# furcelay/gigalens

Hardware: AMD Instinct MI355X
Metric: forward+grad lens sims/sec, 128x128 px batch 1024; achieved HBM GB/s vs peak (higher is better)
Workload: dtype f32; 1 GPU; C2: EPL+shear lens, Sersic source, 128x128 px, batch 1024 per GPU, fp32 (BASELINE.json configs[1]); samples_per_gpu=1024, pixels=16384, z_dim=13, mode=fwdgrad, parallelism=single GPU

## Files before the change

### gigalens_amd/csrc/gigalens_hip.hip

```cpp
#include "../../include/gigalens_hip.h"

#include <hip/hip_runtime.h>

#include <algorithm>
#include <cmath>
#include <cstdarg>
#include <cstdio>
#include <cstdlib>
#include <cstring>
#include <new>
#include <vector>

#define GL_AUX_KERNELS 1
#include "gl_host_tables.h"
#include "gl_model.h"
#include "gl_static.hip.h"
#include "gl_post.hip.h"
#include "gl_positions.hip.h"
#include "gl_images.hip.h"
#include "gl_potential.hip.h"
#include "gl_lstsq.hip.h"
#include "gl_shp.hip.h"

using namespace glk;

namespace {
thread_local char g_err[512] = "";
}

namespace glk {
int fail(int code, const char* fmt, ...) {
  va_list ap;
  va_start(ap, fmt);
  vsnprintf(g_err, sizeof(g_err), fmt, ap);
  va_end(ap);
  return code;
}
}

namespace {

size_t align_up(size_t v, size_t a) { return (v + a - 1) / a * a; }

int env_int(const char* name, int dflt) {
  const char* s = getenv(name);
  return (s && *s) ? atoi(s) : dflt;
}

}


namespace {

void chunking(const gl_model* m, int B, int* chunk, int* n_chunks) {
  const long long tile_px = (long long)WG * 4;
  long long want = std::max<long long>((768 + B - 1) / B, ((long long)m->N + 8191) / 8192);
  if (m->target_wgs_set || !m->static_id) want = std::max<long long>(1, (m->target_wgs + B - 1) / B);
  long long per = ((long long)m->N + want - 1) / want;
  per = std::max(tile_px, (per + tile_px - 1) / tile_px * tile_px);
  if (m->chunk_px_override > 0) per = m->chunk_px_override;
  *chunk = (int)per;
  *n_chunks = (int)(((long long)m->N + per - 1) / per);
}

bool wave_front_end(const gl_model* m) { return m->has_epl && (int)m->comps.size() <= 64 && m->wave_prep; }
bool order_in_front_end(const gl_model* m, int B) {
  return wave_front_end(m) && m->use_order && m->order_fused && m->epl_comp >= 0 && B >= 2;
}

int tail_plan(const gl_model* m, int B, int n_chunks, int* tail_from, int* n_rows) {
  *tail_from = B;
  *n_rows = n_chunks;
  const bool pair_epl = m->pair && (m->static_id == ST_EPLSHEAR_SERSIC || m->static_id == ST_EPLSHEAR_SERSIC_SERSIC);
  if (m->tail_rows == 0 || !pair_epl || m->has_post || !order_in_front_end(m, B) || B > 1024) return 0;
  const int tiles = (m->N + 2 * WG - 1) / (2 * WG);
  const int slots = 256 * (m->static_id == ST_EPLSHEAR_SERSIC ? 3 : 2);
  int n_tail = m->tail_n, rows = m->tail_rows;
  if (n_tail < 0) {
    const long long wgs = (long long)B * n_chunks, rem = wgs % slots;
    if (wgs < slots || rem * 4 < slots) return 0;
    n_tail = (int)(rem / n_chunks);
  }
  if (rows < 0) rows = 2 * n_chunks;
  if (n_tail <= 0 || n_tail > B || rows > tiles || rows == n_chunks) return 0;
  *tail_from = B - n_tail;
  *n_rows = std::max(n_chunks, rows);
  return rows;
}

struct Workspace {
  float* derived;
  float* partial;
  float* params;
  int* order;
  int* cost;
  float* gal_dyn;
  float *pos_w, *pos_adj, *pos_g, *pos_fam, *pos_ll, *pos_chi2, *pos_grad;
  float* img_ss;
  float* img_tmp;
  float* stats;
  size_t bytes;
};

Workspace carve(const gl_model* m, int B, void* base) {
  int chunk, n_chunks;
  chunking(m, B, &chunk, &n_chunks);
  Workspace w{};
  size_t off = 0;
  char* p = (char*)base;
  w.derived = (float*)(p + off);
  off += align_up((size_t)B * m->D * sizeof(float), 256);
  w.partial = (float*)(p + off);
  int tail_from, n_rows;
  tail_plan(m, B, n_chunks, &tail_from, &n_rows);
  off += align_up((size_t)B * n_rows * m->A * sizeof(float), 256);
  w.params = (float*)(p + off);
  off += align_up((size_t)B * std::max(m->P, 1) * sizeof(float), 256);
  w.order = (int*)(p + off);
  off += align_up((size_t)B * sizeof(int), 256);
  w.cost = (int*)(p + off);
  off += align_up((size_t)B * sizeof(int), 256);
  if (m->G) {
    w.gal_dyn = (float*)(p + off);
    off += align_up((size_t)B * m->G * GM_ND * sizeof(float), 256);
  }
  if (m->pos_J) {
    auto take = [&](size_t n) { float* q = (float*)(p + off); off += align_up(n * sizeof(float), 256); return q; };
    w.pos_w = take((size_t)B * m->pos_J * 6);
    w.pos_adj = take((size_t)B * m->pos_J * 3);
    w.pos_g = take((size_t)B * m->pos_J * std::max(m->P, 1));
    w.pos_fam = take((size_t)B * m->pos_F * 2);
    w.pos_ll = take(B);
    w.pos_chi2 = take(B);
    w.pos_grad = take((size_t)B * std::max(m->P, 1));
  }
  if (m->has_post) {
    w.img_ss = (float*)(p + off);
    off += align_up((size_t)B * m->height * m->width * sizeof(float), 256);
    w.img_tmp = (float*)(p + off);
    off += align_up((size_t)B * (m->height / m->supersample) * (m->width / m->supersample) * sizeof(float), 256);
    w.stats = (float*)(p + off);
    off += align_up((size_t)B * 2 * sizeof(float), 256);
  }
  w.bytes = off;
  return w;
}


MainArgs base_args(const gl_model* m, const Workspace& w, int chunk) {
  MainArgs a{};
  a.comps = m->d_comps;
  a.n_lens = m->n_lens;
  a.n_ll = m->n_ll;
  a.n_src = m->n_src;
  a.derived = w.derived;
  a.D = m->D;
  a.A = m->A;
  a.Apad = m->Apad;
  a.ncols = m->ncols;
// ... 494 lines not shown
    int off = NSTAT;
    bool ok_row = true;
    for (int i = 0; i < n_comp; ++i) {
      ok_row = ok_row && m->comps[i].a_off == off;
      off += static_nacc(m->comps[i].kind);
    }
    if (!ok_row || off != m->A) m->pair = 0;
  }
  {
    int off = NSTAT;
    bool ok_row = true;
    for (int i = 0; i < n_comp; ++i) {
      ok_row = ok_row && m->comps[i].a_off == off;
      off += static_nacc(m->comps[i].kind);
    }
    m->shp_kernel = env_int("GIGALENS_HIP_SHP", 1) && env_int("GIGALENS_HIP_PAIR", 1) && m->static_id && ok_row && n_src == 1 &&
                    m->comps.back().kind == K_SHAPELETS;
  }
  m->light_spherical = n_comp > n_lens;
  for (int i = n_lens; i < n_comp; ++i) m->light_spherical = m->light_spherical && m->comps[i].kind == K_SERSIC;
  if (!m->tile_grad) m->tile_grad = m->static_id ? 1 : 2;
  if (!m->static_id) {
    const bool env_tile = env_int("GIGALENS_HIP_TILE", 0) != 0;
    if (!env_tile && !m->has_epl && !m->has_shapelets && !m->fam) m->tile = 4;
    if (m->tile == 1) m->tile = 2;
    if (m->tile_grad == 1) m->tile_grad = 2;
  }
  if (env_int("GIGALENS_HIP_CLUSTER", 1) && !m->static_id && !m->has_user && n_lens_light == 0 && n_lens >= 1 && n_lens <= 8 && n_src >= 1 &&
      n_src <= 20 && (size_t)64 * m->Apad * sizeof(float) <= 64 * 1024) {
    bool ok_c = true, ell = false;
    for (int i = 0; i < n_lens; ++i) ok_c = ok_c && m->comps[i].kind == K_NFW;
    for (int i = n_lens; i < n_comp; ++i) {
      ok_c = ok_c && (m->comps[i].kind == K_SERSIC || m->comps[i].kind == K_SERSIC_ELLIPSE);
      ell = ell || m->comps[i].kind == K_SERSIC_ELLIPSE;
    }
    constexpr int NFWP = (NFW_ND + 3) & ~3, SERP = (SER_NDX + 3) & ~3;
    for (int i = 0; i < n_lens && ok_c; ++i) ok_c = m->comps[i].d_off == NFWP * i && m->comps[i].a_off == NSTAT + NFW_NACC * i;
    for (int i = 0; i < n_src && ok_c; ++i)
      ok_c = m->comps[n_lens + i].d_off == NFWP * n_lens + SERP * i && m->comps[n_lens + i].a_off == NSTAT + NFW_NACC * n_lens + SER_NACC * i;
    ok_c = ok_c && (size_t)64 * m->Apad * sizeof(float) + sizeof(float) * 2 * glh::kNfwNodes <= 64 * 1024;
    if (ok_c) m->cluster = ell ? 2 : 1;
    if (m->cluster) {
      const int cap = (n_lens <= 4 && n_src <= 8) ? 12 : (n_src <= 12 ? 20 : 28);
      const int mode = env_int("GIGALENS_HIP_CLUSTER", -1);
      m->cluster_w = mode == 2 || (mode != 1 && 10 * (n_lens + n_src) >= 6 * cap);
    }
  }
  m->target_wgs = std::max(1, env_int("GIGALENS_HIP_TARGET_WGS", 2048));
  m->target_wgs_set = getenv("GIGALENS_HIP_TARGET_WGS") != nullptr;
  m->use_order = env_int("GIGALENS_HIP_ORDER", 1) != 0;
  m->order_fused = env_int("GIGALENS_HIP_ORDER_FUSED", 1) != 0;
  m->prep_lds = env_int("GIGALENS_HIP_PREP_LDS", 1) != 0;
  m->tail_rows = env_int("GIGALENS_HIP_TAIL_ROWS", -1);
  m->tail_n = env_int("GIGALENS_HIP_TAIL_N", -1);
#ifdef GL_EXPERIMENTS
  m->chunk_px_override = env_int("GIGALENS_HIP_CHUNK_PX", 0);
  m->dbg_flags = env_int("GIGALENS_HIP_DBGFLAGS", 0);
  if (m->chunk_px_override < 0 || m->chunk_px_override % (WG * 4) != 0) {
    const int bad = m->chunk_px_override;
    delete m;
    return fail(GL_EINVAL, "GIGALENS_HIP_CHUNK_PX=%d is not a positive multiple of the tile (%d pixels)", bad, WG * 4);
  }
  if (m->dbg_flags || m->chunk_px_override)
    fprintf(stderr, "libgigalens_hip: EXPERIMENT BUILD with GIGALENS_HIP_DBGFLAGS=%d GIGALENS_HIP_CHUNK_PX=%d -- results are not valid\n",
            m->dbg_flags, m->chunk_px_override);
#else
  for (const char* name : {"GIGALENS_HIP_DBGFLAGS", "GIGALENS_HIP_CHUNK_PX"}) {
    const char* v = getenv(name);
    if (v && *v && atoi(v) != 0) {
      delete m;
      return fail(GL_EINVAL, "%s is set but this library was built without -DGL_EXPERIMENTS (the dissection knobs do not exist in it)", name);
    }
  }
#endif
  m->shp_cull = env_int("GIGALENS_HIP_SHP_CULL", 1);
  m->shp_blocked = env_int("GIGALENS_HIP_SHP_BLOCKED", 1);
  m->corr_max_pairs = env_int("GIGALENS_HIP_CORR_MAXPAIRS", 0);
  m->corr_wide = env_int("GIGALENS_HIP_CORR_WIDE", 1);
  m->wave_prep = env_int("GIGALENS_HIP_WAVE_PREP", 1) != 0;
  m->lstsq_wgs = std::max(1, env_int("GIGALENS_HIP_LSTSQ_WGS", 2048));
  m->lstsq_chol = env_int("GIGALENS_HIP_LSTSQ_CHOL", 1) != 0;
  m->lstsq_fused = env_int("GIGALENS_HIP_LSTSQ_FUSED", 1) != 0;
  size_t shmem = (size_t)(((m->D + 3) & ~3) + m->ncols * m->Apad) * sizeof(float) + m->nfw_lds;
  if (shmem > 64 * 1024) { delete m; return fail(GL_EUNSUPPORTED, "model needs %zu B of LDS per workgroup (> 64 KiB)", shmem); }

  auto up = [&](void** dst, const void* src, size_t bytes) -> bool {
    if (hipMalloc(dst, bytes) != hipSuccess) return false;
    return hipMemcpy(*dst, src, bytes, hipMemcpyHostToDevice) == hipSuccess;
  };
  bool ok = true;
  if (n_comp) ok = ok && up((void**)&m->d_comps, m->comps.data(), sizeof(CompDesc) * n_comp);
  else ok = ok && (hipMalloc((void**)&m->d_comps, sizeof(CompDesc)) == hipSuccess);
  ok = ok && up((void**)&m->d_gx, grid->grid_x, sizeof(float) * m->N);
  for (int i = 0; i < m->N; ++i) m->grid_rmax = std::max(m->grid_rmax, std::hypot(grid->grid_x[i], grid->grid_y[i]));
  ok = ok && up((void**)&m->d_gy, grid->grid_y, sizeof(float) * m->N);
  if (!m->lin_cols.empty()) ok = ok && up((void**)&m->d_lin_cols, m->lin_cols.data(), sizeof(int) * m->lin_cols.size());
  if (grid->pix_index) {
    for (int i = 0; i < m->N && ok; ++i)
      if (grid->pix_index[i] < 0 || grid->pix_index[i] >= m->height * m->width) {
        gl_model_destroy(m);
        return fail(GL_EINVAL, "pix_index[%d]=%d out of range", i, grid->pix_index[i]);
      }
    ok = ok && up((void**)&m->d_pix, grid->pix_index, sizeof(int) * m->N);
  }
  if (m->has_nfw) {
    std::vector<float> tab;
    glh::build_nfw_table([](double X, double& g, double& gp) { glp::nfw_gw<double>(X, g, gp); }, tab);
    const float neutral_nfw[4] = {0.f, 0.f, 1.f, 0.f};
    float neutral_ser[16] = {0.f};
    neutral_ser[glp::SER_C] = neutral_ser[glp::SER_SQ] = neutral_ser[glp::SER_ISQ] = neutral_ser[glp::SER_INVRS] = 1.f;
    neutral_ser[glp::SER_INVN] = neutral_ser[glp::SER_IRS2] = 1.f;
    neutral_ser[glp::SER_BN] = 1.6721f;
    tab.insert(tab.end(), neutral_nfw, neutral_nfw + 4);
    tab.insert(tab.end(), neutral_ser, neutral_ser + 16);
    std::vector<float> tab_s;
    glh::build_nfw_table_s([](double X, double& g, double& gp) { glp::nfw_gw<double>(X, g, gp); }, tab_s);
    tab.insert(tab.end(), tab_s.begin(), tab_s.end());
    ok = ok && up((void**)&m->d_nfw_tab, tab.data(), tab.size() * sizeof(float));
  }
  if (m->has_table) {
    std::vector<float> tab;
    (void)sh_nmax;
    glh::build_shapelet_table(m->shp_big ? SH_CAPB : SH_CAP, tab, &m->shp_stride);
    ok = ok && up((void**)&m->d_shp_tab, tab.data(), tab.size() * sizeof(float));
  }
  m->has_post = grid->psf != nullptr || grid->supersample != 1;
  if (m->has_post) {
    const int kh = grid->psf ? grid->psf_h : 1, kw = grid->psf ? grid->psf_w : 1, ss = grid->supersample;
    m->psf_h = kh;
    m->psf_w = kw;
    m->KH = kh + ss - 1;
    m->KW = kw + ss - 1;
    m->pad_t = (kh - 1) / 2;
    m->pad_l = (kw - 1) / 2;
    std::vector<double> keff((size_t)m->KH * m->KW, 0.0);
    for (int u = 0; u < kh; ++u)
      for (int v = 0; v < kw; ++v) {
        double f = grid->psf ? (double)grid->psf[(size_t)(kh - 1 - u) * kw + (kw - 1 - v)] : 1.0;
        for (int a2 = 0; a2 < ss; ++a2)
          for (int c2 = 0; c2 < ss; ++c2) keff[(size_t)(u + a2) * m->KW + (v + c2)] += f / (double)(ss * ss);
      }
    std::vector<float> kf(keff.begin(), keff.end());
    ok = ok && up((void**)&m->d_psf, kf.data(), sizeof(float) * kf.size());
    if (env_int("GIGALENS_HIP_CORR_PAIR", 1) && ss <= 2 && m->KW <= 32 && m->KH <= 64) {
      const int Hs = m->height, Ws = m->width, H = Hs / ss, W = Ws / ss;
      std::vector<float> kbuf;
      auto pad4 = [](int n) { return std::max(4, (n + 3) & ~3); };
      {
        gl_model::CorrPlan& f = m->corr_fwd;
        f.KWP = pad4(m->KW);
        f.ST = ss;
        CorrClass c{};
        c.koff = 0; c.KH = m->KH; c.pt = m->pad_t; c.pl = m->pad_l; c.Ho = H; c.Wo[0] = W; c.oo_r = 0; c.oo_c[0] = 0;
        kbuf.assign((size_t)m->KH * f.KWP, 0.f);
        for (int u = 0; u < m->KH; ++u)
          for (int v = 0; v < m->KW; ++v) kbuf[(size_t)u * f.KWP + v] = (float)keff[(size_t)u * m->KW + v];
        f.args.n_class = 1; f.args.ncj = 1; f.args.Hi = Hs; f.args.Wi = Ws; f.args.Hout = H; f.args.Wout = W; f.args.os = 1;
        f.args.cls[0] = c;
        f.max_Ho = H; f.max_Wo = W; f.max_KH = m->KH; f.ok = true;
      }
      {
        gl_model::CorrPlan& g = m->corr_bwd;
        g.ST = 1;
        g.args.n_class = ss; g.args.ncj = ss; g.args.Hi = H; g.args.Wi = W; g.args.Hout = Hs; g.args.Wout = Ws; g.args.os = ss;
        int Cn[4], rjn[4], pln[4], max_pl = -(1 << 30), width = 1;
        for (int pj = 0; pj < ss; ++pj) {
// ... 1118 lines not shown
```

### gigalens_amd/csrc/gl_launch.hip.h

```cpp
#pragma once
#include <hip/hip_ext.h>

#include "gl_model.h"
#include "gl_static.hip.h"
#include "gl_pair.hip.h"
#include "gl_shp.hip.h"

namespace glk {

template <int MODE>
bool launch_static(const gl_model* m, const MainArgs& a, dim3 grid, dim3 block, size_t shmem, hipStream_t stream, hipEvent_t ev0, hipEvent_t ev1) {
  const int T = (MODE == IMG_BWD || MODE == LL_GRAD) ? m->tile_grad : m->tile;
#define GL_PAIR(WW, LK, CK, SK)                                                           \
  do {                                                                                    \
    m->last_main_fn = (const void*)&gl_pair_kernel<MODE, v2f, WW, LK, CK, SK>;            \
    hipExtLaunchKernelGGL((gl_pair_kernel<MODE, v2f, WW, LK, CK, SK>), grid, block, (std::uint32_t)(shmem), stream, ev0, ev1, 0, a); \
  } while (0)
  if (m->pair) {
    constexpr bool G = (MODE == IMG_BWD || MODE == LL_GRAD);
    constexpr int W1 = G ? 3 : 4, W2 = G ? 2 : 4;
    if (m->light_spherical) {
      switch (m->static_id) {
        case ST_EPLSHEAR_SERSIC: GL_PAIR(W1, L_EplShear, C_None, C_Sersic); return true;
        case ST_EPLSHEAR_SERSIC_SERSIC: GL_PAIR(W2, L_EplShear, C_Sersic, C_Sersic); return true;
        case ST_SIE_SERSIC: GL_PAIR(W1, L_Sie, C_None, C_Sersic); return true;
        case ST_SIESHEAR_SERSIC_SERSIC: GL_PAIR(W1, L_SieShear, C_Sersic, C_Sersic); return true;
        default: break;
      }
    } else {
      switch (m->static_id) {
        case ST_EPLSHEAR_SERSIC: GL_PAIR(W1, L_EplShear, C_None, C_SersicE); return true;
        case ST_EPLSHEAR_SERSIC_SERSIC: GL_PAIR(W2, L_EplShear, C_SersicE, C_SersicE); return true;
        case ST_SIE_SERSIC: GL_PAIR(W1, L_Sie, C_None, C_SersicE); return true;
        case ST_SIESHEAR_SERSIC_SERSIC: GL_PAIR(W2, L_SieShear, C_SersicE, C_SersicE); return true;
        default: break;
      }
    }
  }
#undef GL_PAIR
  if (m->shp_kernel && (m->static_id == ST_EPLSHEAR_SHAPELETS || m->static_id == ST_EPLSHEAR_SERSIC_SHAPELETS)) {
    constexpr int NPS = SH_SQ / 2;
    const size_t epi = (size_t)(16 * m->Apad + 4 * 16 * 17) * sizeof(float);
    const size_t sh = (size_t)((m->D + 3) & ~3) * sizeof(float) + std::max(shp_exchange_bytes(NPS), epi);
    const bool interp = (m->comps.back().flags & GL_FLAG_SHAPELETS_INTERPOLATE) != 0;
    const bool ragged = a.mask || a.pix || (a.N % (2 * WG)) != 0 || (a.chunk % (2 * WG)) != 0;
    MainArgs ab = a;
    ab.blk_w = (interp && !ragged && m->shp_blocked && m->width % 16 == 0 && m->height % 8 == 0 &&
                (long long)a.N == (long long)m->width * m->height) ? m->width : 0;
#define GL_SHP2(LLK_, I_, R_)                                                                                 \
  do {                                                                                                        \
    m->last_main_fn = (const void*)&gl_shp_kernel<MODE, 2, L_EplShear, LLK_, NPS, I_, R_>;                     \
    hipExtLaunchKernelGGL((gl_shp_kernel<MODE, 2, L_EplShear, LLK_, NPS, I_, R_>), grid, block, (std::uint32_t)(sh), stream, ev0, ev1, 0, ab);   \
  } while (0)
#define GL_SHP(LLK_, I_) do { if (ragged) GL_SHP2(LLK_, I_, true); else GL_SHP2(LLK_, I_, false); } while (0)
    if (m->static_id == ST_EPLSHEAR_SHAPELETS) { if (interp) GL_SHP(C_None, true); else GL_SHP(C_None, false); }
    else { if (interp) GL_SHP(C_SersicE, true); else GL_SHP(C_SersicE, false); }
#undef GL_SHP
#undef GL_SHP2
    return true;
  }
#define GL_LAUNCH(TT, WW, LK, CK, SK)                                                        \
  do {                                                                                       \
    m->last_main_fn = (const void*)&gl_static_kernel<MODE, TT, WW, LK, CK, SK>;              \
    hipExtLaunchKernelGGL((gl_static_kernel<MODE, TT, WW, LK, CK, SK>), grid, block, (std::uint32_t)(shmem), stream, ev0, ev1, 0, a); \
  } while (0)
  switch (m->static_id) {
    case ST_EPLSHEAR_SERSIC:
      if (T == 4) { if (m->static_variant == 2) GL_LAUNCH(4, 2, L_EplShear, C_None, C_Sersic); else GL_LAUNCH(4, 3, L_EplShear, C_None, C_Sersic); }
      else if (T == 1) GL_LAUNCH(1, 4, L_EplShear, C_None, C_Sersic);
      else { if (m->static_variant == 3) GL_LAUNCH(2, 3, L_EplShear, C_None, C_Sersic); else GL_LAUNCH(2, 4, L_EplShear, C_None, C_Sersic); }
      return true;
    case ST_EPLSHEAR_SERSIC_SERSIC:
      if (T == 4) GL_LAUNCH(4, 2, L_EplShear, C_Sersic, C_Sersic); else GL_LAUNCH(2, 4, L_EplShear, C_Sersic, C_Sersic);
      return true;
    case ST_SIE_SERSIC:
      if (T == 4) GL_LAUNCH(4, 4, L_Sie, C_None, C_Sersic); else GL_LAUNCH(2, 4, L_Sie, C_None, C_Sersic);
      return true;
    case ST_SIESHEAR_SERSIC_SERSIC:
      if (T == 4) GL_LAUNCH(4, 4, L_SieShear, C_Sersic, C_Sersic); else GL_LAUNCH(2, 4, L_SieShear, C_Sersic, C_Sersic);
      return true;
    case ST_EPLSHEAR_SHAPELETS:
      if (T == 2) GL_LAUNCH(2, 2, L_EplShear, C_None, C_Shapelets); else if (T == 1) GL_LAUNCH(1, 2, L_EplShear, C_None, C_Shapelets);
      else return false;
      return true;
    case ST_EPLSHEAR_SERSIC_SHAPELETS:
      if (T == 2) GL_LAUNCH(2, 2, L_EplShear, C_Sersic, C_Shapelets); else if (T == 1) GL_LAUNCH(1, 2, L_EplShear, C_Sersic, C_Shapelets);
      else return false;
      return true;
  }
#undef GL_LAUNCH
  return false;
}

template <int MODE>
int launch_generic(const gl_model* m, const MainArgs& a, dim3 grid, dim3 block, size_t shmem, hipStream_t stream, hipEvent_t ev0, hipEvent_t ev1);

template <int MODE>
int launch_main(const gl_model* m, const MainArgs& a, int B, int n_chunks, hipStream_t stream) {
  dim3 grid(n_chunks, B), block(WG);
  if (a.tail_rows > 0)
    grid.y = a.tail_from + (unsigned)(((long long)(B - a.tail_from) * a.tail_rows + n_chunks - 1) / n_chunks);
  size_t shmem = (size_t)(((m->D + 3) & ~3) + m->ncols * m->Apad) * sizeof(float) + m->nfw_lds;
  const bool timed = m->timing_slots && (m->timing_calls.fetch_add(1) % m->timing_stride) == 0;
// ... 22 lines not shown
```

### gigalens_amd/csrc/gl_pair.hip.h

```cpp
#pragma once
#include "gl_static.hip.h"
#include "gl_vec.hip.h"

namespace glk {

#ifdef GL_HAVE_USER
template <class V, int CODE> __device__ __forceinline__ void user_mass_fwd_v(const float* d, V x, V y, V& bx, V& by) {
  constexpr unsigned body = (unsigned)user_code_body(CODE);
  if constexpr (sizeof(V) == sizeof(float)) {
    float ax, ay;
    glu::mass_fwd(body, d, x, y, ax, ay);
    bx -= ax; by -= ay;
  } else {
    float ax0, ay0, ax1, ay1;
    glu::mass_fwd(body, d, x.x, y.x, ax0, ay0);
    glu::mass_fwd(body, d, x.y, y.y, ax1, ay1);
    bx -= V{ax0, ax1};
    by -= V{ay0, ay1};
  }
}
template <class V, int CODE> __device__ __forceinline__ void user_mass_vjp_v(const float* d, V x, V y, V gx, V gy, V* acc) {
  constexpr unsigned body = (unsigned)user_code_body(CODE);
  constexpr int NPAR = user_code_npar(CODE);
  float t0[NPAR > 0 ? NPAR : 1], t1[NPAR > 0 ? NPAR : 1];
#pragma unroll
  for (int k = 0; k < NPAR; ++k) { t0[k] = 0.f; t1[k] = 0.f; }
  if constexpr (sizeof(V) == sizeof(float)) {
    glu::mass_vjp(body, d, x, y, gx, gy, t0);
#pragma unroll
    for (int k = 0; k < NPAR; ++k) acc[k] += t0[k];
  } else {
    glu::mass_vjp(body, d, x.x, y.x, gx.x, gy.x, t0);
    glu::mass_vjp(body, d, x.y, y.y, gx.y, gy.y, t1);
#pragma unroll
    for (int k = 0; k < NPAR; ++k) acc[k] += V{t0[k], t1[k]};
  }
}
template <class V, int CODE> __device__ __forceinline__ V user_light_fwd_v(const float* d, V x, V y) {
  constexpr unsigned body = (unsigned)user_code_body(CODE);
  if constexpr (sizeof(V) == sizeof(float)) return glu::light_fwd(body, d, x, y);
  else return V{glu::light_fwd(body, d, x.x, y.x), glu::light_fwd(body, d, x.y, y.y)};
}
template <class V, int CODE, bool SRC>
__device__ __forceinline__ void user_light_vjp_v(const float* d, V x, V y, V g, V* acc, V& gpx, V& gpy) {
  constexpr unsigned body = (unsigned)user_code_body(CODE);
  constexpr int NPAR = user_code_npar(CODE);
  float t0[NPAR > 0 ? NPAR : 1], t1[NPAR > 0 ? NPAR : 1];
#pragma unroll
  for (int k = 0; k < NPAR; ++k) { t0[k] = 0.f; t1[k] = 0.f; }
  if constexpr (sizeof(V) == sizeof(float)) {
    float dgx = 0.f, dgy = 0.f;
    glu::light_vjp(body, d, x, y, g, t0, dgx, dgy);
#pragma unroll
    for (int k = 0; k < NPAR; ++k) acc[k] += t0[k];
    if (SRC) { gpx += dgx; gpy += dgy; }
  } else {
    float dgx0 = 0.f, dgy0 = 0.f, dgx1 = 0.f, dgy1 = 0.f;
    glu::light_vjp(body, d, x.x, y.x, g.x, t0, dgx0, dgy0);
    glu::light_vjp(body, d, x.y, y.y, g.y, t1, dgx1, dgy1);
#pragma unroll
    for (int k = 0; k < NPAR; ++k) acc[k] += V{t0[k], t1[k]};
    if (SRC) { gpx += V{dgx0, dgx1}; gpy += V{dgy0, dgy1}; }
  }
}
#endif

template <int MODE, class V, int WAVES, class LK, class LLK, class SK>
__global__ void __launch_bounds__(WG, WAVES) gl_pair_kernel(MainArgs a) {
  constexpr int NL = LK::n, NLL = LLK::n, NS = SK::n, NLIGHT = NLL + NS;
  constexpr bool GRAD = (MODE == IMG_BWD || MODE == LL_GRAD);
  constexpr int W = sizeof(V) / sizeof(float);
  extern __shared__ float smem[];
  float* s_d = smem;
  float* s_acc = smem + ((a.D + 3) & ~3);
  const int tid = threadIdx.x;
  int rank = blockIdx.y, row = blockIdx.x, n_rows = gridDim.x, my_rows = gridDim.x;
  int p0 = row * a.chunk, p1 = min(p0 + a.chunk, a.N);
  if (a.tail_rows > 0) {
    n_rows = a.n_rows;
    if (rank >= a.tail_from) {
      const int j = (rank - a.tail_from) * (int)gridDim.x + row;
      rank = a.tail_from + j / a.tail_rows;
      if (rank >= a.n_samples) return;
      row = j % a.tail_rows;
      my_rows = a.tail_rows;
      const int tiles = (a.N + W * WG - 1) / (W * WG);
      p0 = (int)((long long)row * tiles / a.tail_rows) * (W * WG);
      p1 = min((int)((long long)(row + 1) * tiles / a.tail_rows) * (W * WG), a.N);
    }
  }
  const int b = a.order ? a.order[rank] : rank;
  const CompDesc* __restrict__ comps = a.comps;
  const float* __restrict__ gder = a.derived + (size_t)b * a.D;
  if (!GL_DBG(a.dbg, 4)) {
    if (a.D <= WG) {
      if (tid < a.D) s_d[tid] = gder[tid];
    } else {
      for (int i = tid; i < a.D; i += WG) s_d[i] = gder[i];
    }
  }
  __syncthreads();
  constexpr int NACC_L = [] { int n = 0; for (int i = 0; i < NL; ++i) n += static_nacc(LK::kinds[i]); return n; }();
  constexpr int NACC_C = [] {
    int n = 0;
    for (int i = 0; i < NLL; ++i) n += static_nacc(LLK::kinds[i]);
    for (int i = 0; i < NS; ++i) n += static_nacc(SK::kinds[i]);
    return n;
  }();
  V accL[NACC_L > 0 ? NACC_L : 1];
  V accC[NACC_C > 0 ? NACC_C : 1];
#pragma unroll
  for (int k = 0; k < NACC_L; ++k) accL[k] = V(0.f);
#pragma unroll
  for (int k = 0; k < NACC_C; ++k) accC[k] = V(0.f);
  V st0 = V(0.f), st1 = V(0.f);
  V wsum = V(0.f);
  int n_whole = 0;
  const float* dL[NL > 0 ? NL : 1];
  const float* dC[NLIGHT > 0 ? NLIGHT : 1];
#pragma unroll
  for (int i = 0; i < NL; ++i) dL[i] = s_d + comps[i].d_off;
#pragma unroll
  for (int i = 0; i < NLIGHT; ++i) dC[i] = s_d + comps[NL + i].d_off;
  const bool has_err = a.err != nullptr, has_mask = a.mask != nullptr, has_pix = a.pix != nullptr;

  auto tile = [&](int base, auto check_tag, auto err_tag) {
    constexpr bool CHECK = decltype(check_tag)::value;
    constexpr int ERR = decltype(err_tag)::value;
    const bool herr = ERR == 2 ? has_err : ERR == 1;
    unsigned jj[W], pidx[W];
    bool valid[W];
    V x, y, vmask = V(1.f);
#pragma unroll
    for (int w = 0; w < W; ++w) {
      int j = base + w * WG + tid;
      valid[w] = CHECK ? (j < p1) : true;
      jj[w] = (unsigned)(valid[w] ? j : p1 - 1);
      pidx[w] = (CHECK && has_pix) ? (unsigned)a.pix[jj[w]] : jj[w];
    }
    unsigned jo[W], po[W];
#pragma unroll
    for (int w = 0; w < W; ++w) { jo[w] = jj[w] << 2; po[w] = pidx[w] << 2; }
    auto ldf = [](const float* base, unsigned byte_off) { return *reinterpret_cast<const float*>(reinterpret_cast<const char*>(base) + byte_off); };
    if constexpr (W == 2) {
      x = V{ldf(a.gx, jo[0]), ldf(a.gx, jo[1])};
      y = V{ldf(a.gy, jo[0]), ldf(a.gy, jo[1])};
      if (CHECK) vmask = V{valid[0] ? 1.f : 0.f, valid[1] ? 1.f : 0.f};
    } else {
      x = ldf(a.gx, jo[0]);
      y = ldf(a.gy, jo[0]);
      if (CHECK) vmask = valid[0] ? 1.f : 0.f;
    }
    V bx = x, by = y, m = V(0.f);
    EplStateV<V> est[NL > 0 ? NL : 1];
    SerStateV<V> sst[NLIGHT > 0 ? NLIGHT : 1];
    static_for([&](auto I) {
      constexpr int i = decltype(I)::value;
      constexpr int kind = LK::kinds[i];
      if constexpr (kind == K_EPL) epl_fwd_v<V, GRAD>(dL[i], gder + comps[i].d_off, x, y, bx, by, est[i]);
      else if constexpr (kind == K_SIE) sie_fwd_v<V>(dL[i], x, y, bx, by);
      else if constexpr (kind == K_SHEAR) shear_fwd_v<V>(dL[i], x, y, bx, by);
#ifdef GL_HAVE_USER
      else if constexpr (is_user_code(kind)) user_mass_fwd_v<V, kind>(dL[i], x, y, bx, by);
#endif
      else sis_fwd_v<V>(dL[i], x, y, bx, by);
    }, std::make_integer_sequence<int, NL>{});
    static_for([&](auto I) {
      constexpr int i = decltype(I)::value;
      constexpr bool src = i >= NLL;
      constexpr int lkind = src ? SK::kinds[src ? i - NLL : 0] : LLK::kinds[src ? 0 : i];
      constexpr bool ell = lkind != K_SERSIC;
#ifdef GL_HAVE_USER
      if constexpr (is_user_code(lkind)) m += user_light_fwd_v<V, lkind>(dC[i], src ? bx : x, src ? by : y);
      else
#endif
      m += sersic_fwd_v<V, ell>(dC[i], src ? bx : x, src ? by : y, sst[i]);
    }, std::make_integer_sequence<int, NLIGHT>{});
    auto nanp = m != m;
    m = (nanp ? V(0.f) : m) * a.out_scale;
    if (MODE == IMG_FWD) {
      float* row = a.img + (size_t)b * a.img_stride;
      if constexpr (W == 2) {
        if (valid[0]) row[pidx[0]] = m.x;
        if (valid[1]) row[pidx[1]] = m.y;
      } else {
        if (valid[0]) row[pidx[0]] = m;
      }
      return;
    }
    V gm;
    if (MODE == IMG_BWD) {
      const float* row = a.gimg + (size_t)b * a.img_stride;
      V g;
      if constexpr (W == 2) g = V{row[pidx[0]], row[pidx[1]]}; else g = row[pidx[0]];
      gm = nanp ? V(0.f) : (CHECK ? g * vmask : g) * a.out_scale;
    } else {
      V o, w = vmask, e = V(1.f);
      if constexpr (W == 2) {
        o = V{ldf(a.obs, po[0]), ldf(a.obs, po[1])};
        if (CHECK && has_mask) w = w * V{ldf(a.mask, po[0]), ldf(a.mask, po[1])};
        if (herr) e = V{ldf(a.err, po[0]), ldf(a.err, po[1])};
      } else {
        o = ldf(a.obs, po[0]);
        if (CHECK && has_mask) w = w * ldf(a.mask, po[0]);
        if (herr) e = ldf(a.err, po[0]);
      }
      V dmo = m - o;
      V s2 = herr ? e * e : m * a.inv_t + a.bg2;
      V is2 = rcp(s2);
      V nm = log2_(s2);
      V c2 = __builtin_elementwise_fma(nm, V(0.f), dmo * dmo * is2);
      if (CHECK) {
        auto use = w != V(0.f);
        st0 += use ? c2 * w : V(0.f);
        st1 += use ? nm * w : V(0.f);
        wsum += w;
      } else {
        st0 += c2;
        st1 += nm;
      }
      if (MODE == LL_GRAD) {
        V g = herr ? -(dmo * is2) : (dmo * dmo * is2 - 1.f) * (is2 * (0.5f * a.inv_t)) - dmo * is2;
        gm = nanp ? V(0.f) : (CHECK ? g * w : g) * a.out_scale;
      }
    }
    if constexpr (GRAD) {
      V gbx = V(0.f), gby = V(0.f);
      static_for([&](auto I) {
        constexpr int i = decltype(I)::value;
        constexpr bool src = i >= NLL;
        constexpr int off = [] {
          int n = 0;
          for (int j = 0; j < i; ++j) n += static_nacc(j < NLL ? LLK::kinds[j < NLL ? j : 0] : SK::kinds[j >= NLL ? j - NLL : 0]);
          return n;
        }();
        constexpr int lkind = src ? SK::kinds[src ? i - NLL : 0] : LLK::kinds[src ? 0 : i];
        constexpr bool ell = lkind != K_SERSIC;
#ifdef GL_HAVE_USER
        if constexpr (is_user_code(lkind)) user_light_vjp_v<V, lkind, src>(dC[i], src ? bx : x, src ? by : y, gm, accC + off, gbx, gby);
        else
#endif
        sersic_vjp_v<V, src, ell>(dC[i], sst[i], gm, accC + off, gbx, gby);
      }, std::make_integer_sequence<int, NLIGHT>{});
      gbx = -gbx;
      gby = -gby;
      static_for([&](auto I) {
        constexpr int i = decltype(I)::value;
        constexpr int kind = LK::kinds[i];
        constexpr int off = [] { int n = 0; for (int j = 0; j < i; ++j) n += static_nacc(LK::kinds[j]); return n; }();
        if constexpr (kind == K_EPL) epl_vjp_v<V>(dL[i], gbx, gby, est[i], accL + off);
        else if constexpr (kind == K_SIE) sie_vjp_v<V>(dL[i], x, y, gbx, gby, accL + off);
        else if constexpr (kind == K_SHEAR) shear_vjp_v<V>(x, y, gbx, gby, accL + off);
#ifdef GL_HAVE_USER
        else if constexpr (is_user_code(kind)) user_mass_vjp_v<V, kind>(dL[i], x, y, gbx, gby, accL + off);
#endif
        else sis_vjp_v<V>(dL[i], x, y, gbx, gby, accL + off);
      }, std::make_integer_sequence<int, NL>{});
    }
  };
  {
    const bool plain = !has_mask && !has_pix;
    int base = p0;
    if (GL_DBG(a.dbg, 1)) base = p1;
    if (plain) {
      if (has_err)
        for (; base + WG * W <= p1; base += WG * W, ++n_whole) tile(base, std::false_type{}, std::integral_constant<int, 1>{});
      else
        for (; base + WG * W <= p1; base += WG * W, ++n_whole) tile(base, std::false_type{}, std::integral_constant<int, 0>{});
    }
    for (; base < p1; base += WG * W) tile(base, std::true_type{}, std::integral_constant<int, 2>{});
  }
  if (MODE == IMG_FWD) return;
  auto norm_term = [](float l2sum, float w) { return (l2sum + w * 2.6514961294723187f) * (float)kLn2; };
  float* out = a.partial + ((size_t)b * n_rows + row) * a.A;
  if (row == 0)
    for (int i = my_rows * a.A + tid; i < n_rows * a.A; i += WG) out[i] = 0.f;
  if (!GRAD) {
    for (int i = tid; i < 4 * a.Apad; i += WG) s_acc[i] = 0.f;
    __syncthreads();
  }
  if constexpr (GRAD) {
    constexpr int NV = NSTAT + NACC_L + NACC_C, NVP = (NV + 3) & ~3;
    float vals[NVP];
#pragma unroll
    for (int k = 0; k < NVP; ++k) vals[k] = 0.f;
    vals[0] = (MODE == LL_GRAD) ? hsum(st0) : 0.f;
    vals[1] = (MODE == LL_GRAD) ? norm_term(hsum(st1), hsum(wsum) + (float)(W * n_whole)) : 0.f;
    static_for([&](auto I) {
      constexpr int i = decltype(I)::value;
      constexpr int kind = LK::kinds[i];
      constexpr int off = [] { int n = 0; for (int j = 0; j < i; ++j) n += static_nacc(LK::kinds[j]); return n; }();
      constexpr int G = static_nacc(kind);
      float tmp[G];
#pragma unroll
      for (int k = 0; k < G; ++k) tmp[k] = hsum(accL[off + k]);
      if constexpr (kind == K_EPL) {
        tmp[EPLA_B] = tmp[EPLA_P0] * (dL[i][EPL_TM1] * dL[i][EPL_INVB]);
        tmp[EPLA_P0] *= rcp(dL[i][EPL_P0]);
        const float gxr = tmp[EPLA_CX], gyr = tmp[EPLA_CY], cc = dL[i][EPL_C], ss = dL[i][EPL_S];
        tmp[EPLA_CX] = -(gxr * cc - gyr * ss);
        tmp[EPLA_CY] = -(gxr * ss + gyr * cc);
      }
#pragma unroll
      for (int k = 0; k < G; ++k) vals[NSTAT + off + k] = tmp[k];
    }, std::make_integer_sequence<int, NL>{});
    static_for([&](auto I) {
      constexpr int i = decltype(I)::value;
      constexpr int off = [] {
        int n = 0;
        for (int j = 0; j < i; ++j) n += static_nacc(j < NLL ? LLK::kinds[j < NLL ? j : 0] : SK::kinds[j >= NLL ? j - NLL : 0]);
        return n;
      }();
      constexpr int lkind = i < NLL ? LLK::kinds[i < NLL ? i : 0] : SK::kinds[i >= NLL ? i - NLL : 0];
      if constexpr (is_user_code(lkind)) {
#pragma unroll
        for (int k = 0; k < static_nacc(lkind); ++k) vals[NSTAT + NACC_L + off + k] = hsum(accC[off + k]);
      } else {
#pragma unroll
        for (int k = 0; k < SER_NACC; ++k) vals[NSTAT + NACC_L + off + k] = hsum(accC[off + k]) * (k == SERA_INVN ? (float)kLn2 : 1.f);
      }
    }, std::make_integer_sequence<int, NLIGHT>{});
    const bool odd = tid & 1, hi = tid & 2;
    float* s_row16 = s_acc + (tid >> 4) * a.Apad;
#pragma unroll
    for (int g = 0; g < NVP / 4; ++g) {
      float r = quad_transpose_sum(vals[4 * g], vals[4 * g + 1], vals[4 * g + 2], vals[4 * g + 3], odd, hi);
      r = dpp_add(r, 0x114, 0xF);
      r = dpp_add(r, 0x118, 0xF);
      if ((tid & 15) >= 12 && 4 * g + (tid & 3) < NV) s_row16[4 * g + (tid & 3)] = r;
    }
    __syncthreads();
    for (int k = tid; k < NV; k += WG) {
      float v = 0.f;
#pragma unroll
// ... 22 lines not shown
```

### gigalens_amd/csrc/gl_static.hip.h

```cpp
#pragma once
#if defined(__HIPCC_RTC__) && !__has_include(<utility>)
namespace std {
template <class T, T v> struct integral_constant {
  static constexpr T value = v;
  typedef T value_type;
  typedef integral_constant type;
  constexpr operator T() const { return v; }
};
typedef integral_constant<bool, true> true_type;
typedef integral_constant<bool, false> false_type;
template <class T, T... Is> struct integer_sequence {};
template <class T, T N> using make_integer_sequence = __make_integer_seq<integer_sequence, T, N>;
template <bool B, class T, class F> struct conditional { typedef T type; };
template <class T, class F> struct conditional<false, T, F> { typedef F type; };
template <bool B, class T, class F> using conditional_t = typename conditional<B, T, F>::type;
}
#else
#include <utility>
#endif

#include "gl_kernels.hip.h"
#include "gl_shapelets.hip.h"

namespace glk {
// ... 312 lines not shown
          return n;
        }();
        const float* d = dC[i];
#pragma unroll
        for (int t = 0; t < T; ++t) {
          float dgx = 0.f, dgy = 0.f;
          if constexpr (kind == K_SHAPELETS)
            shp_vjp_state<SH_CAP>(d, gder + comps[NL + i].d_off + SHP_AMP, comps[NL + i].flags & 1u, hst[i][t], gm[t],
                                  accC + off, dgx, dgy);
          else
            sersic_vjp_state(d, sst[i][t], gm[t], accC + off, dgx, dgy);
          if (src) { gbx[t] += dgx; gby[t] += dgy; }
        }
      }, std::make_integer_sequence<int, NLIGHT>{});
#pragma unroll
      for (int t = 0; t < T; ++t) { gbx[t] = -gbx[t]; gby[t] = -gby[t]; }
      static_for([&](auto I) {
        constexpr int i = decltype(I)::value;
        constexpr int kind = LK::kinds[i];
        constexpr int off = [] { int n = 0; for (int j = 0; j < i; ++j) n += static_nacc(LK::kinds[j]); return n; }();
        const float* d = dL[i];
        if constexpr (kind == K_EPL) {
          epl_vjp_state<T>(d, gbx, gby, est[i], accL + off);
        } else {
#pragma unroll
          for (int t = 0; t < T; ++t) {
            if constexpr (kind == K_SIE) sie_vjp(d, x[t], y[t], gbx[t], gby[t], accL + off);
            else if constexpr (kind == K_NFW) nfw_vjp(d, x[t], y[t], gbx[t], gby[t], accL + off);
            else if constexpr (kind == K_SHEAR) shear_vjp(d, x[t], y[t], gbx[t], gby[t], accL + off);
            else sis_vjp(d, x[t], y[t], gbx[t], gby[t], accL + off);
          }
        }
      }, std::make_integer_sequence<int, NL>{});
    }
  }
  if (MODE == IMG_FWD) return;
  const AccCol ac = acc_col(s_acc, a.Apad, a.ncols, tid);
  if (MODE == LL_FWD || MODE == LL_GRAD) wave_acc<2>(st, ac, 0);
  if constexpr (GRAD) {
    static_for([&](auto I) {
      constexpr int i = decltype(I)::value;
      constexpr int off = [] { int n = 0; for (int j = 0; j < i; ++j) n += static_nacc(LK::kinds[j]); return n; }();
      constexpr int G = static_nacc(LK::kinds[i]);
      float tmp[G];
#pragma unroll
      for (int k = 0; k < G; ++k) tmp[k] = accL[off + k];
      wave_acc<G>(tmp, ac, comps[i].a_off, comps[i].n_acc);
    }, std::make_integer_sequence<int, NL>{});
    static_for([&](auto I) {
      constexpr int i = decltype(I)::value;
      constexpr int kind = i < NLL ? LLK::kinds[i < NLL ? i : 0] : SK::kinds[i >= NLL ? i - NLL : 0];
      constexpr int off = [] {
        int n = 0;
        for (int j = 0; j < i; ++j) n += static_nacc(j < NLL ? LLK::kinds[j < NLL ? j : 0] : SK::kinds[j >= NLL ? j - NLL : 0]);
        return n;
      }();
      constexpr int G = static_nacc(kind);
      float tmp[G];
#pragma unroll
      for (int k = 0; k < G; ++k) tmp[k] = accC[off + k];
      wave_acc<G>(tmp, ac, comps[NL + i].a_off, comps[NL + i].n_acc);
    }, std::make_integer_sequence<int, NLIGHT>{});
  }
  __syncthreads();
  float* out = a.partial + ((size_t)b * gridDim.x + chunk) * a.A;
  for (int k = tid; k < a.A; k += WG) {
    float v = 0.f;
    for (int j = 0; j < a.ncols; ++j) v += s_acc[j * a.Apad + k];
    out[k] = v;
  }
}

using L_EplShear = KindList<K_EPL, K_SHEAR>;
using L_Sie = KindList<K_SIE>;
using L_SieShear = KindList<K_SIE, K_SHEAR>;
using C_None = KindList<>;
using C_Sersic = KindList<K_SERSIC>;
using C_SersicE = KindList<K_SERSIC_ELLIPSE>;
using C_Shapelets = KindList<K_SHAPELETS>;

enum StaticId { ST_NONE = 0, ST_EPLSHEAR_SERSIC, ST_EPLSHEAR_SERSIC_SERSIC, ST_SIE_SERSIC, ST_EPLSHEAR_SHAPELETS,
                ST_SIESHEAR_SERSIC_SERSIC, ST_EPLSHEAR_SERSIC_SHAPELETS  };


}
```

### gigalens_amd/csrc/gl_vec.hip.h

```cpp
#pragma once
#include <hip/hip_runtime.h>

#include "gl_profiles.h"

namespace glk {
using namespace glp;

typedef float v2f __attribute__((ext_vector_type(2)));

using glm::rcp;
using glm::sqrt_;
using glm::exp2_;
using glm::log2_;
using glm::atan_;
using glm::atanh_;

__device__ __forceinline__ v2f rcp(v2f a) { return v2f{glm::rcp(a.x), glm::rcp(a.y)}; }
__device__ __forceinline__ v2f sqrt_(v2f a) { return v2f{glm::sqrt_(a.x), glm::sqrt_(a.y)}; }
__device__ __forceinline__ float rsq_(float a) { return __builtin_amdgcn_rsqf(a); }
__device__ __forceinline__ v2f rsq_(v2f a) { return v2f{__builtin_amdgcn_rsqf(a.x), __builtin_amdgcn_rsqf(a.y)}; }
__device__ __forceinline__ v2f exp2_(v2f a) { return v2f{glm::exp2_(a.x), glm::exp2_(a.y)}; }
__device__ __forceinline__ v2f log2_(v2f a) { return v2f{glm::log2_(a.x), glm::log2_(a.y)}; }
__device__ __forceinline__ v2f atan_(v2f a) { return v2f{glm::atan_(a.x), glm::atan_(a.y)}; }
__device__ __forceinline__ v2f atanh_(v2f a) { return v2f{glm::atanh_(a.x), glm::atanh_(a.y)}; }
template <class V> __device__ __forceinline__ V vexp(V x) {
  const float hi = (float)kLog2e;
  const float lo = (float)(kLog2e - (double)(float)kLog2e);
  V t = x * hi;
  V e = __builtin_elementwise_fma(x, V(hi), -t) + x * lo;
  V p = exp2_(t);
  return __builtin_elementwise_fma(p, e * (float)kLn2, p);
}
template <> __device__ __forceinline__ float vexp<float>(float x) { return glm::exp_(x); }
template <class V> __device__ __forceinline__ V vlog(V x) { return log2_(x) * (float)kLn2; }
__device__ __forceinline__ float floor_at(float a, float lo) { return __builtin_fmaxf(a, lo); }
__device__ __forceinline__ v2f floor_at(v2f a, float lo) { return v2f{__builtin_fmaxf(a.x, lo), __builtin_fmaxf(a.y, lo)}; }
__device__ __forceinline__ float clamp3(float a, float lo, float hi) { return __builtin_amdgcn_fmed3f(a, lo, hi); }
__device__ __forceinline__ v2f clamp3(v2f a, float lo, float hi) { return v2f{__builtin_amdgcn_fmed3f(a.x, lo, hi), __builtin_amdgcn_fmed3f(a.y, lo, hi)}; }
template <class V> __device__ __forceinline__ V vmin(V a, V b) { return a < b ? a : b; }
template <class V> __device__ __forceinline__ V vmax(V a, V b) { return a > b ? a : b; }
__device__ __forceinline__ float hsum(float a) { return a; }
__device__ __forceinline__ float hsum(v2f a) { return a.x + a.y; }

template <class V> struct EplStateV {
  V xr, yr, inv, invc, L2, P, Cs, Ss, arx, ary;
  V f0, f1, t0, t1;
};

typedef const float __attribute__((address_space(4)))* gptr4;
typedef float vf4 __attribute__((ext_vector_type(4)));
template <class T, class P> struct gl_rebind;
template <class T> struct gl_rebind<T, const float*> { using type = const T*; };
template <class T> struct gl_rebind<T, gptr4> { using type = const T __attribute__((address_space(4)))*; };

template <class V, bool GRAD, class P = const float*>
__device__ __forceinline__ void epl_fwd_v(const float* d, const P gd, V x, V y, V& bx, V& by,
                                          EplStateV<V>& st) {
  using PInt = typename gl_rebind<int, P>::type;
  using PRow = typename gl_rebind<vf4, P>::type;
  const float c = d[EPL_C], s = d[EPL_S], q = d[EPL_Q];
  V dx = x - d[EPL_CX], dy = y - d[EPL_CY];
  st.xr = dx * c + dy * s;
  st.yr = dy * c - dx * s;
  V X = st.xr * q;
  V r2 = X * X + st.yr * st.yr;
  V r = rsq_(r2);
  auto pos = r2 > V(0.f);
  st.inv = pos ? r : V(0.f);
  st.Cs = pos ? X * r : V(1.f);
  st.Ss = st.yr * st.inv;
  V iRc = clamp3(r, 1e-10f, 1e10f);
  st.invc = (iRc == r) ? r : V(0.f);
  V twoc = (st.Cs * st.Cs - st.Ss * st.Ss) * 2.f;
  const int K = ((PInt)gd)[EPL_KI];
  const PRow gtab = (PRow)(gd + EPL_TAB);
  V o1, o2, f1 = V(0.f), f2 = V(0.f), t1 = V(0.f), t2 = V(0.f);
  auto term = [&](const vf4 ck, V& b1, V& b2, V& g1, V& g2, V& h1, V& h2) {
    b2 = __builtin_elementwise_fma(twoc, b1, V(ck.x)) - b2;
    if (GRAD) {
      g2 = __builtin_elementwise_fma(twoc, g1, V(ck.z)) - g2;
      h2 = __builtin_elementwise_fma(twoc, h1, V(ck.w)) - h2;
    }
  };
  auto four = [&](const vf4 r0, const vf4 r1, const vf4 r2, const vf4 r3) {
    term(r3, o1, o2, f1, f2, t1, t2);
    term(r2, o2, o1, f2, f1, t2, t1);
    term(r1, o1, o2, f1, f2, t1, t2);
    term(r0, o2, o1, f2, f1, t2, t1);
  };
  auto four_first = [&](const vf4 r0, const vf4 r1, const vf4 r2, const vf4 r3) {
    o1 = __builtin_elementwise_fma(twoc, V(r3.x), V(r2.x));
    o2 = __builtin_elementwise_fma(twoc, o1, V(r1.x)) - V(r3.x);
    o1 = __builtin_elementwise_fma(twoc, o2, V(r0.x)) - o1;
    if (GRAD) {
      f1 = __builtin_elementwise_fma(twoc, V(r3.z), V(r2.z));
      f2 = __builtin_elementwise_fma(twoc, f1, V(r1.z)) - V(r3.z);
      f1 = __builtin_elementwise_fma(twoc, f2, V(r0.z)) - f1;
      t1 = __builtin_elementwise_fma(twoc, V(r3.w), V(r2.w));
      t2 = __builtin_elementwise_fma(twoc, t1, V(r1.w)) - V(r3.w);
      t1 = __builtin_elementwise_fma(twoc, t2, V(r0.w)) - t1;
    }
  };
  int trips = (K + 4) >> 2;
  int row = 4 * trips - 4;
  PRow p = gtab + row;
  vf4 a0 = p[0], a1 = p[1], a2 = p[2], a3 = p[3];
  row = row >= 4 ? row - 4 : 0;
  p = gtab + row;
  vf4 b0 = p[0], b1 = p[1], b2 = p[2], b3 = p[3];
  four_first(a0, a1, a2, a3);
  if (--trips != 0) {
    while (true) {
      row = row >= 4 ? row - 4 : 0;
      p = gtab + row;
      a0 = p[0]; a1 = p[1]; a2 = p[2]; a3 = p[3];
      four(b0, b1, b2, b3);
      if (--trips == 0) break;
      row = row >= 4 ? row - 4 : 0;
      p = gtab + row;
      b0 = p[0]; b1 = p[1]; b2 = p[2]; b3 = p[3];
      four(a0, a1, a2, a3);
      if (--trips == 0) break;
    }
  }
  const V o0 = o1, ob = o2;
  if (GRAD) { st.f0 = f1; st.f1 = f2; st.t0 = t1; st.t1 = t2; }
  const V Ox = (o0 - ob) * st.Cs, Oy = (o0 + ob) * st.Ss;
  st.L2 = log2_(iRc * d[EPL_B]);
  st.P = exp2_(st.L2 * d[EPL_TM1]) * d[EPL_P0];
  const V arx = st.P * Ox, ary = st.P * Oy;
// ... 219 lines not shown
```

Baseline: 12.41 million sims/s.

## Park EPL series state in LDS to raise gradient pair-kernel occupancy

In the gradient pair kernel for EPL+shear+Sersic, four EPL state vectors (f0,f1,t0,t1) are stored to LDS after the forward pass and reloaded before the VJP. This frees registers so launch bounds can target one more wave per SIMD (3 to 4). The host chunking and tail planning now use the larger resident round, and the LDS request grows by the park buffer. The cost is extra LDS traffic and footprint per workgroup, and the compiler may spill if the tighter register budget is not met.

```diff
diff --git a/gigalens_amd/csrc/gigalens_hip.hip b/gigalens_amd/csrc/gigalens_hip.hip
--- a/gigalens_amd/csrc/gigalens_hip.hip
+++ b/gigalens_amd/csrc/gigalens_hip.hip
@@ -52,9 +52,12 @@
 
 namespace {
 
+int resident_round(const gl_model* m) { return 256 * (m->pair ? pair_grad_resident(m->static_id, m->light_spherical) : 3); }
+
 void chunking(const gl_model* m, int B, int* chunk, int* n_chunks) {
   const long long tile_px = (long long)WG * 4;
-  long long want = std::max<long long>((768 + B - 1) / B, ((long long)m->N + 8191) / 8192);
+  const int round = std::max(resident_round(m), 768);
+  long long want = std::max<long long>((round + B - 1) / B, ((long long)m->N + 8191) / 8192);
   if (m->target_wgs_set || !m->static_id) want = std::max<long long>(1, (m->target_wgs + B - 1) / B);
   long long per = ((long long)m->N + want - 1) / want;
   per = std::max(tile_px, (per + tile_px - 1) / tile_px * tile_px);
@@ -74,7 +77,7 @@
   const bool pair_epl = m->pair && (m->static_id == ST_EPLSHEAR_SERSIC || m->static_id == ST_EPLSHEAR_SERSIC_SERSIC);
   if (m->tail_rows == 0 || !pair_epl || m->has_post || !order_in_front_end(m, B) || B > 1024) return 0;
   const int tiles = (m->N + 2 * WG - 1) / (2 * WG);
-  const int slots = 256 * (m->static_id == ST_EPLSHEAR_SERSIC ? 3 : 2);
+  const int slots = resident_round(m);
   int n_tail = m->tail_n, rows = m->tail_rows;
   if (n_tail < 0) {
     const long long wgs = (long long)B * n_chunks, rem = wgs % slots;
@@ -735,6 +738,8 @@
   m->lstsq_chol = env_int("GIGALENS_HIP_LSTSQ_CHOL", 1) != 0;
   m->lstsq_fused = env_int("GIGALENS_HIP_LSTSQ_FUSED", 1) != 0;
   size_t shmem = (size_t)(((m->D + 3) & ~3) + m->ncols * m->Apad) * sizeof(float) + m->nfw_lds;
+  if (m->pair && pair_grad_resident(m->static_id, m->light_spherical) > pair_grad_class(m->static_id, m->light_spherical))
+    shmem += (size_t)EPL_PARK_N * WG * 2 * sizeof(float);
   if (shmem > 64 * 1024) { delete m; return fail(GL_EUNSUPPORTED, "model needs %zu B of LDS per workgroup (> 64 KiB)", shmem); }
 
   auto up = [&](void** dst, const void* src, size_t bytes) -> bool {
diff --git a/gigalens_amd/csrc/gl_launch.hip.h b/gigalens_amd/csrc/gl_launch.hip.h
--- a/gigalens_amd/csrc/gl_launch.hip.h
+++ b/gigalens_amd/csrc/gl_launch.hip.h
@@ -14,11 +14,15 @@
 #define GL_PAIR(WW, LK, CK, SK)                                                           \
   do {                                                                                    \
     m->last_main_fn = (const void*)&gl_pair_kernel<MODE, v2f, WW, LK, CK, SK>;            \
-    hipExtLaunchKernelGGL((gl_pair_kernel<MODE, v2f, WW, LK, CK, SK>), grid, block, (std::uint32_t)(shmem), stream, ev0, ev1, 0, a); \
+    hipExtLaunchKernelGGL((gl_pair_kernel<MODE, v2f, WW, LK, CK, SK>), grid, block,                                                  \
+                          (std::uint32_t)(shmem + pair_park_bytes<MODE, v2f, WW, LK>()), stream, ev0, ev1, 0, a);                    \
   } while (0)
   if (m->pair) {
     constexpr bool G = (MODE == IMG_BWD || MODE == LL_GRAD);
-    constexpr int W1 = G ? 3 : 4, W2 = G ? 2 : 4;
+    constexpr int W1 = G ? pair_grad_class(ST_EPLSHEAR_SERSIC, true) : 4, W2 = G ? pair_grad_class(ST_EPLSHEAR_SERSIC_SERSIC, true) : 4;
+    static_assert(!G || (pair_waves<MODE, v2f, W1, L_EplShear>() == pair_grad_resident(ST_EPLSHEAR_SERSIC, true) &&
+                         pair_waves<MODE, v2f, W2, L_EplShear>() == pair_grad_resident(ST_EPLSHEAR_SERSIC_SERSIC, true)),
+                  "the kernels' waves per SIMD and the host's resident round disagree");
     if (m->light_spherical) {
       switch (m->static_id) {
         case ST_EPLSHEAR_SERSIC: GL_PAIR(W1, L_EplShear, C_None, C_Sersic); return true;
diff --git a/gigalens_amd/csrc/gl_pair.hip.h b/gigalens_amd/csrc/gl_pair.hip.h
--- a/gigalens_amd/csrc/gl_pair.hip.h
+++ b/gigalens_amd/csrc/gl_pair.hip.h
@@ -65,15 +65,35 @@
 }
 #endif
 
+template <class LK> constexpr int pair_n_epl() { int n = 0; for (int i = 0; i < LK::n; ++i) n += LK::kinds[i] == K_EPL; return n; }
+template <int MODE, class V, int WAVES, class LK> constexpr bool pair_parked() {
+  return pair_parks(MODE == IMG_BWD || MODE == LL_GRAD, (int)(sizeof(V) / sizeof(float)), WAVES, pair_n_epl<LK>() > 0);
+}
+template <int MODE, class V, int WAVES, class LK> constexpr int pair_waves() { return WAVES + (pair_parked<MODE, V, WAVES, LK>() ? 1 : 0); }
+template <int MODE, class V, int WAVES, class LK> constexpr size_t pair_park_bytes() {
+  return pair_parked<MODE, V, WAVES, LK>() ? (size_t)pair_n_epl<LK>() * EPL_PARK_N * WG * sizeof(V) : 0;
+}
+
 template <int MODE, class V, int WAVES, class LK, class LLK, class SK>
-__global__ void __launch_bounds__(WG, WAVES) gl_pair_kernel(MainArgs a) {
+__global__ void __launch_bounds__(WG, (pair_waves<MODE, V, WAVES, LK>())) gl_pair_kernel(MainArgs a) {
   constexpr int NL = LK::n, NLL = LLK::n, NS = SK::n, NLIGHT = NLL + NS;
   constexpr bool GRAD = (MODE == IMG_BWD || MODE == LL_GRAD);
+  constexpr bool PARK = pair_parked<MODE, V, WAVES, LK>();
+  constexpr auto epl_ordinal = [](int i) { int n = 0; for (int j = 0; j < i; ++j) n += LK::kinds[j] == K_EPL; return n; };
   constexpr int W = sizeof(V) / sizeof(float);
   extern __shared__ float smem[];
   float* s_d = smem;
   float* s_acc = smem + ((a.D + 3) & ~3);
   const int tid = threadIdx.x;
+  V* park_wr = nullptr;
+  const V* park_rd = nullptr;
+  if constexpr (PARK) {
+    V* park = reinterpret_cast<V*>(s_acc + a.ncols * a.Apad);
+    int rd = tid;
+    asm("" : "+v"(rd));
+    park_wr = park + tid;
+    park_rd = park + rd;
+  }
   int rank = blockIdx.y, row = blockIdx.x, n_rows = gridDim.x, my_rows = gridDim.x;
   int p0 = row * a.chunk, p1 = min(p0 + a.chunk, a.N);
   if (a.tail_rows > 0) {
@@ -157,8 +177,10 @@
     static_for([&](auto I) {
       constexpr int i = decltype(I)::value;
       constexpr int kind = LK::kinds[i];
-      if constexpr (kind == K_EPL) epl_fwd_v<V, GRAD>(dL[i], gder + comps[i].d_off, x, y, bx, by, est[i]);
-      else if constexpr (kind == K_SIE) sie_fwd_v<V>(dL[i], x, y, bx, by);
+      if constexpr (kind == K_EPL) {
+        epl_fwd_v<V, GRAD>(dL[i], gder + comps[i].d_off, x, y, bx, by, est[i]);
+        if constexpr (PARK) epl_park<WG>(est[i], park_wr + epl_ordinal(i) * EPL_PARK_N * WG);
+      } else if constexpr (kind == K_SIE) sie_fwd_v<V>(dL[i], x, y, bx, by);
       else if constexpr (kind == K_SHEAR) shear_fwd_v<V>(dL[i], x, y, bx, by);
 #ifdef GL_HAVE_USER
       else if constexpr (is_user_code(kind)) user_mass_fwd_v<V, kind>(dL[i], x, y, bx, by);
@@ -248,8 +270,10 @@
         constexpr int i = decltype(I)::value;
         constexpr int kind = LK::kinds[i];
         constexpr int off = [] { int n = 0; for (int j = 0; j < i; ++j) n += static_nacc(LK::kinds[j]); return n; }();
-        if constexpr (kind == K_EPL) epl_vjp_v<V>(dL[i], gbx, gby, est[i], accL + off);
-        else if constexpr (kind == K_SIE) sie_vjp_v<V>(dL[i], x, y, gbx, gby, accL + off);
+        if constexpr (kind == K_EPL) {
+          if constexpr (PARK) epl_unpark<WG>(est[i], park_rd + epl_ordinal(i) * EPL_PARK_N * WG);
+          epl_vjp_v<V>(dL[i], gbx, gby, est[i], accL + off);
+        } else if constexpr (kind == K_SIE) sie_vjp_v<V>(dL[i], x, y, gbx, gby, accL + off);
         else if constexpr (kind == K_SHEAR) shear_vjp_v<V>(x, y, gbx, gby, accL + off);
 #ifdef GL_HAVE_USER
         else if constexpr (is_user_code(kind)) user_mass_vjp_v<V, kind>(dL[i], x, y, gbx, gby, accL + off);
diff --git a/gigalens_amd/csrc/gl_static.hip.h b/gigalens_amd/csrc/gl_static.hip.h
--- a/gigalens_amd/csrc/gl_static.hip.h
+++ b/gigalens_amd/csrc/gl_static.hip.h
@@ -418,5 +418,15 @@
 enum StaticId { ST_NONE = 0, ST_EPLSHEAR_SERSIC, ST_EPLSHEAR_SERSIC_SERSIC, ST_SIE_SERSIC, ST_EPLSHEAR_SHAPELETS,
                 ST_SIESHEAR_SERSIC_SERSIC, ST_EPLSHEAR_SERSIC_SHAPELETS  };
 
-
-}
+constexpr int pair_grad_class(int static_id, bool light_spherical) {
+  return static_id == ST_EPLSHEAR_SERSIC_SERSIC ? 2 : (static_id == ST_SIESHEAR_SERSIC_SERSIC && !light_spherical) ? 2 : 3;
+}
+constexpr bool pair_parks(bool grad, int lanes, int waves_class, bool has_epl) { return grad && lanes == 2 && waves_class == 3 && has_epl; }
+constexpr int pair_grad_resident(int static_id, bool light_spherical) {
+  const bool epl = static_id == ST_EPLSHEAR_SERSIC || static_id == ST_EPLSHEAR_SERSIC_SERSIC;
+  const int c = pair_grad_class(static_id, light_spherical);
+  return c + (pair_parks(true, 2, c, epl) ? 1 : 0);
+}
+
+
+}
diff --git a/gigalens_amd/csrc/gl_vec.hip.h b/gigalens_amd/csrc/gl_vec.hip.h
--- a/gigalens_amd/csrc/gl_vec.hip.h
+++ b/gigalens_amd/csrc/gl_vec.hip.h
@@ -46,6 +46,14 @@
   V xr, yr, inv, invc, L2, P, Cs, Ss, arx, ary;
   V f0, f1, t0, t1;
 };
+
+constexpr int EPL_PARK_N = 4;
+template <int STRIDE, class V> __device__ __forceinline__ void epl_park(const EplStateV<V>& st, V* slot) {
+  slot[0 * STRIDE] = st.f0; slot[1 * STRIDE] = st.f1; slot[2 * STRIDE] = st.t0; slot[3 * STRIDE] = st.t1;
+}
+template <int STRIDE, class V> __device__ __forceinline__ void epl_unpark(EplStateV<V>& st, const V* slot) {
+  st.f0 = slot[0 * STRIDE]; st.f1 = slot[1 * STRIDE]; st.t0 = slot[2 * STRIDE]; st.t1 = slot[3 * STRIDE];
+}
 
 typedef const float __attribute__((address_space(4)))* gptr4;
 typedef float vf4 __attribute__((ext_vector_type(4)));
```

New measurement: 11.85 million sims/s (median of 2 runs). -4.5%, worse.
